# 0xPolygonZero/plonky2

Hardware: NVIDIA H100
Metric: goldilocks_field_elements_per_s_ntt_lde_merkle (higher is better)
Workload: dtype u64

## Files before the change

### plonky2_b200/csrc/gl_lazy.cuh

```cuda
#pragma once
#include "gl_field.cuh"

namespace gl {

struct L3 {
    uint32_t w0, w1;
    int32_t e;
};

GL_HD L3 l3_from(uint64_t x) { return L3{(uint32_t)x, (uint32_t)(x >> 32), 0}; }

#if defined(__CUDA_ARCH__)
__device__ __forceinline__ L3 l3_add(L3 a, L3 b) {
    L3 r;
    asm("add.cc.u32 %0, %3, %6;\n\taddc.cc.u32 %1, %4, %7;\n\taddc.u32 %2, %5, %8;"
        : "=r"(r.w0), "=r"(r.w1), "=r"(r.e)
        : "r"(a.w0), "r"(a.w1), "r"(a.e), "r"(b.w0), "r"(b.w1), "r"(b.e));
    return r;
}
__device__ __forceinline__ L3 l3_sub(L3 a, L3 b) {
    L3 r;
    asm("sub.cc.u32 %0, %3, %6;\n\tsubc.cc.u32 %1, %4, %7;\n\tsubc.u32 %2, %5, %8;"
        : "=r"(r.w0), "=r"(r.w1), "=r"(r.e)
        : "r"(a.w0), "r"(a.w1), "r"(a.e), "r"(b.w0), "r"(b.w1), "r"(b.e));
// ... 66 lines not shown
    return r;
}
inline L3 l3_add(L3 a, L3 b) { return l3_of(l3_val(a) + l3_val(b)); }
inline L3 l3_sub(L3 a, L3 b) { return l3_of(l3_val(a) - l3_val(b)); }
inline uint64_t l3_norm(L3 a) {
    __int128 v = l3_val(a) % (__int128)P;
    if (v < 0) v += P;
    return (uint64_t)v;
}
template <int S>
inline L3 l3_shift(L3 a) { return l3_from(mul_pow2(l3_norm(a), (uint32_t)S)); }
#endif

template <int S>
GL_HD L3 l3_shift_c(L3 a) { return l3_shift<S>(a); }
template <int M, int L, int B>
struct DftLazyBfly {
    static GL_HD void run(L3* r) {
        constexpr int half = 1 << (M - 1 - L);
        constexpr int j = B % half, blk = (B / half) * 2 * half;
        constexpr int sh = (96 / half) * j;
        const L3 u = r[blk + j], v = r[blk + j + half];
        r[blk + j] = l3_add(u, v);
        r[blk + j + half] = l3_shift_c<sh>(l3_sub(u, v));
        if constexpr (B + 1 < (1 << (M - 1))) DftLazyBfly<M, L, B + 1>::run(r);
        else if constexpr (L + 1 < M) DftLazyBfly<M, L + 1, 0>::run(r);
    }
};
template <int M>
GL_HD void dft_lazy(L3* r) {
    if constexpr (M > 0) DftLazyBfly<M, 0, 0>::run(r);
}

}
```

### plonky2_b200/csrc/gl_ntt.cuh

```cuda
#pragma once
#include "gl_lazy.cuh"

namespace gl {

constexpr int NTT_MAX_LOG_PASS = 10;
constexpr int NTT_COL_MIN_LOG = 5;

GL_HD constexpr int ntt_r2(int log) { return log / 2; }
GL_HD constexpr int ntt_r1(int log) { return log - log / 2; }

template <int LOG>
struct PassCfg {
    static constexpr int R1 = ntt_r1(LOG), R2 = ntt_r2(LOG);
    static constexpr int E = 1 << R1, TPT = 1 << R2, NSUB = E / TPT;
    static constexpr int ROW_THREADS = (TPT * 8 < 32) ? 32 : TPT * 8;
    static constexpr int LPC = ROW_THREADS / TPT;
    static constexpr int ROW_MIN_BLOCKS = (E >= 32 ? 512 : 768) / ROW_THREADS;
    static constexpr int ROW_PITCH = TPT + 1;
    static constexpr int ROW_S_WORDS = E * ROW_PITCH;
    static constexpr int GATHER_PITCH = (1 << LOG) + 2;
    static constexpr int T = (256 / TPT) < 8 ? 8 : (256 / TPT);
    static constexpr int COL_THREADS = T * TPT;
    static constexpr int COL_MIN_BLOCKS = (E >= 32 ? 512 : 768) / COL_THREADS;
    static constexpr int COL_QPITCH = TPT * T + 8;
    static constexpr int COL_S_WORDS = E * COL_QPITCH;
};
GL_HD constexpr size_t ntt_row_smem_bytes(int log, bool natural) {
    const int r1 = ntt_r1(log), r2 = ntt_r2(log), E = 1 << r1, TPT = 1 << r2;
    const int threads = (TPT * 8 < 32) ? 32 : TPT * 8, lpc = threads / TPT;
    const size_t s = (size_t)lpc * E * (TPT + 1), g = natural ? (size_t)lpc * ((1 << log) + 2) : 0;
    return (s > g ? s : g) * 8;
}
GL_HD constexpr size_t ntt_col_smem_bytes(int log) {
    const int r1 = ntt_r1(log), r2 = ntt_r2(log), E = 1 << r1, TPT = 1 << r2;
    const int T = (256 / TPT) < 8 ? 8 : (256 / TPT);
    return (size_t)E * (TPT * T + 8) * 8;
}

GL_HD uint64_t table_step_entry(int log, uint32_t idx, uint64_t scale, uint64_t base) {
    const int r1 = ntt_r1(log), r2 = ntt_r2(log);
    const uint32_t t = idx & ((1u << r2) - 1), q = idx >> r2;
    const uint64_t k = bitrev32(q, (uint32_t)r1);
    uint64_t v = pow(root_of_unity((uint32_t)log), k * t);
    if (base != 1) v = mul(v, pow(base, t));
    if (scale != 1) v = mul(v, scale);
    return v;
}
GL_HD uint64_t table_post_entry(int a, int b, size_t idx, uint64_t base) {
    const size_t p = idx >> b, j2 = idx & (((size_t)1 << b) - 1);
    const uint64_t k1 = bitrev32((uint32_t)p, (uint32_t)a);
    uint64_t v = pow(root_of_unity((uint32_t)(a + b)), k1 * j2);
    if (base != 1) v = mul(v, pow(base, j2));
    return v;
}

template <int LOG>
GL_HD void pass_step1(uint64_t* x, const uint64_t* tw, const uint64_t* uq, bool tw_full, int t) {
    using Cf = PassCfg<LOG>;
    L3 r[Cf::E];
#pragma unroll
    for (int q = 0; q < Cf::E; q++) {
        uint64_t v = x[q];
// ... 105 lines not shown
    return cp.twa + (p << cp.log_c) + (size_t)tile * Cf::T + tt;
}
template <int LOG>
GL_HD void col_phase2_store(const ColPass& cp, int blk, int tid, const uint64_t* z, const uint64_t* tws, size_t stride_j,
                            size_t stride_m) {
    using Cf = PassCfg<LOG>;
    const int tt = tid % Cf::T, t = tid / Cf::T;
    size_t in_off, out_off;
    int tile;
    col_unit<LOG>(cp, blk, in_off, out_off, tile);
    const size_t C = (size_t)1 << cp.log_c;
    uint64_t* dst = cp.out + out_off + (size_t)tile * Cf::T + tt;
#pragma unroll
    for (int m = 0; m < Cf::NSUB; m++) {
#pragma unroll
        for (int j = 0; j < Cf::TPT; j++) {
            const int i = m * Cf::TPT + j;
            const size_t p = (size_t)(t + Cf::TPT * m) * Cf::TPT + j;
            dst[p * C] = mul(z[i], tws[m * stride_m + j * stride_j]);
        }
    }
}
template <int LOG>
GL_HD void col_phase2(const ColPass& cp, const uint64_t* S, int blk, int tid) {
    using Cf = PassCfg<LOG>;
    if (Cf::R2 == 0) return;
    uint64_t z[Cf::E];
    col_phase2_load<LOG>(S, tid, z);
    col_phase2_dft<LOG>(z);
    const size_t C = (size_t)1 << cp.log_c;
    col_phase2_store<LOG>(cp, blk, tid, z, col_twiddle_src<LOG>(cp, blk, tid, 0), C, (size_t)Cf::TPT * Cf::TPT * C);
}

enum RowMode { RM_BITREV = 0, RM_NATURAL = 1 };
struct RowPass {
    const uint64_t* in;
    uint64_t* out;
    size_t in_stride, out_stride;
    const uint64_t* tw;
    int log_r;
    int ncols;
    int tw_full;
    int has_uq;
    int reverse;
    size_t row0;
    int n_peer;
    uint64_t* out_peer[7];
    uint64_t uq[32];
};
template <int LOG, int MODE>
GL_HD bool row_line(const RowPass& rp, int blk, int l, size_t& col, size_t& prow, size_t& kbase) {
    using Cf = PassCfg<LOG>;
    const size_t L = (size_t)blk * Cf::LPC + l;
    const size_t R = (size_t)1 << rp.log_r;
    col = L >> rp.log_r;
    const size_t low = L & (R - 1);
    if (MODE == RM_BITREV) {
        prow = low;
        kbase = 0;
    } else {
        kbase = low;
        prow = rp.log_r ? (size_t)bitrev32((uint32_t)low, (uint32_t)rp.log_r) : 0;
    }
    return col < (size_t)rp.ncols;
}
template <int LOG>
GL_HD int row_blocks(const RowPass& rp) {
    using Cf = PassCfg<LOG>;
    const size_t lines = (size_t)rp.ncols << rp.log_r;
    return (int)((lines + Cf::LPC - 1) / Cf::LPC);
}
template <int LOG, int MODE>
GL_HD void row_load(const RowPass& rp, int blk, int tid, uint64_t* x) {
    using Cf = PassCfg<LOG>;
    const int l = tid / Cf::TPT, t = tid % Cf::TPT;
    size_t col, prow, kbase;
    const bool live = row_line<LOG, MODE>(rp, blk, l, col, prow, kbase);
    const uint64_t* src = rp.in + col * rp.in_stride + (prow << LOG) + t;
#pragma unroll
    for (int q = 0; q < Cf::E; q++) x[q] = live ? src[Cf::TPT * q] : 0;
}
template <int LOG, int MODE>
GL_HD void row_phase1(const RowPass& rp, uint64_t* S, int blk, int tid, uint64_t* x) {
    using Cf = PassCfg<LOG>;
    const int l = tid / Cf::TPT, t = tid % Cf::TPT;
    pass_step1<LOG>(x, rp.tw, rp.has_uq ? rp.uq : nullptr, rp.tw_full != 0, t);
    if (Cf::R2 == 0) return;
    uint64_t* Sl = S + (size_t)l * Cf::ROW_S_WORDS;
#pragma unroll
    for (int q = 0; q < Cf::E; q++) Sl[q * Cf::ROW_PITCH + t] = x[q];
}
template <int LOG>
GL_HD uint32_t row_natural_index(int q, int j) {
    using Cf = PassCfg<LOG>;
    return bitrev32((uint32_t)q, Cf::R1) + (uint32_t)Cf::E * (Cf::R2 ? bitrev32((uint32_t)j, Cf::R2) : 0u);
}
template <int LOG>
GL_HD void row_phase2_load(const uint64_t* S, int tid, int m, uint64_t* z) {
    using Cf = PassCfg<LOG>;
    const int l = tid / Cf::TPT, t = tid % Cf::TPT;
    const uint64_t* Sl = S + (size_t)l * Cf::ROW_S_WORDS;
    const int q = t + Cf::TPT * m;
#pragma unroll
// ... 139 lines not shown
```

### plonky2_b200/csrc/gl_ntt_host.cuh

```cuda
#pragma once

template <int LOG, bool ASYNC_TW>
__global__ void __launch_bounds__(PassCfg<LOG>::COL_THREADS, PassCfg<LOG>::COL_MIN_BLOCKS) k_ntt_col(ColPass cp) {
    using Cf = PassCfg<LOG>;
    extern __shared__ __align__(16) u64 smem[];
    u64* tw_s = smem;
    u64* S = smem + (1 << LOG);
    u64* mbar = S + Cf::COL_S_WORDS;
    tma_table_issue(tw_s, cp.tw, (uint32_t)((1 << LOG) * 8), mbar);
    u64 x[Cf::E];
    col_load<LOG>(cp, blockIdx.x, threadIdx.x, x);
    __syncthreads();
    ColPass c2 = cp;
    c2.tw = tw_s;
    tma_table_wait(mbar);
    col_phase1<LOG>(c2, S, blockIdx.x, threadIdx.x, x);
    if (Cf::R2 == 0) return;
    __syncthreads();
    if (!ASYNC_TW) {
        col_phase2<LOG>(c2, S, blockIdx.x, threadIdx.x);
        return;
    }
    col_phase2_load<LOG>(S, threadIdx.x, x);
    __syncthreads();
// ... 48 lines not shown
            if (!(q == 0 && skip0)) y = mul(y, twp[(size_t)q * tws]);
            x[q] = y;
        }
        if (s == 0) {
#pragma unroll
            for (int q = 0; q < Cf::E; q++) S[q * Cf::COL_QPITCH + t * Cf::T + tt] = x[q];
            __syncthreads();
#pragma unroll
            for (int j = 0; j < Cf::TPT; j++) x[j] = S[t * Cf::COL_QPITCH + j * Cf::T + tt];
            skip0 = false;
            const u64* tw2 = cp.twa + (((size_t)t * Cf::TPT) << cp.log_c) + (size_t)tile * Cf::T + tt;
            if (ASYNC_TW) {
                __syncthreads();
#pragma unroll
                for (int j = 0; j < Cf::TPT; j++)
                    asm volatile("cp.async.ca.shared.global [%0], [%1], 8;" ::"r"(smem_u32(S + col_twiddle_slot<LOG>(threadIdx.x, j))),
                                 "l"(tw2 + (size_t)j * C)
                                 : "memory");
                asm volatile("cp.async.commit_group;" ::: "memory");
                twp = S + col_twiddle_slot<LOG>(threadIdx.x, 0);
                tws = Cf::COL_THREADS;
            } else {
                twp = tw2;
                tws = C;
            }
        }
    }
    u64* dst = cp.out + out_off + (size_t)tile * Cf::T + tt;
#pragma unroll
    for (int j = 0; j < Cf::TPT; j++) dst[((size_t)t * Cf::TPT + j) * C] = x[j];
}

template <int LOG, int MODE>
__global__ void __launch_bounds__(PassCfg<LOG>::ROW_THREADS, PassCfg<LOG>::ROW_MIN_BLOCKS) k_ntt_row(RowPass rp) {
    using Cf = PassCfg<LOG>;
    extern __shared__ __align__(16) u64 smem[];
    u64* tw_s = smem;
    u64* S = smem + (1 << LOG);
    u64* mbar = S + ntt_row_smem_bytes(LOG, MODE == RM_NATURAL) / 8;
    RowPass r2 = rp;
    u64 x[Cf::E];
    if (Cf::R2 > 0 && LOG >= 4) {
        tma_table_issue(tw_s, rp.tw, (uint32_t)((1 << LOG) * 8), mbar);
        row_load<LOG, MODE>(rp, blockIdx.x, threadIdx.x, x);
        __syncthreads();
        r2.tw = tw_s;
        tma_table_wait(mbar);
    } else {
        row_load<LOG, MODE>(rp, blockIdx.x, threadIdx.x, x);
    }
    row_phase1<LOG, MODE>(r2, S, blockIdx.x, threadIdx.x, x);
    if (Cf::R2 == 0) {
        if (MODE == RM_BITREV) {
            row_store_bitrev<LOG>(r2, blockIdx.x, threadIdx.x, 0, x);
        } else {
            row_gather_write<LOG>(S, threadIdx.x, 0, x);
            __syncthreads();
            row_store_natural<LOG>(r2, S, blockIdx.x, threadIdx.x, blockDim.x);
        }
        return;
    }
    __syncwarp();
    if (MODE == RM_BITREV) {
#pragma unroll
        for (int m = 0; m < Cf::NSUB; m++) {
            u64 z[Cf::TPT];
            row_phase2_load<LOG>(S, threadIdx.x, m, z);
            pass_step2<LOG>(z);
            row_store_bitrev<LOG>(r2, blockIdx.x, threadIdx.x, m, z);
        }
    } else {
        u64 z[Cf::NSUB][Cf::TPT];
#pragma unroll
        for (int m = 0; m < Cf::NSUB; m++) {
            row_phase2_load<LOG>(S, threadIdx.x, m, z[m]);
            pass_step2<LOG>(z[m]);
        }
        __syncthreads();
#pragma unroll
        for (int m = 0; m < Cf::NSUB; m++) row_gather_write<LOG>(S, threadIdx.x, m, z[m]);
        __syncthreads();
        row_store_natural<LOG>(r2, S, blockIdx.x, threadIdx.x, blockDim.x);
    }
}

template <int LOG, int MODE>
__global__ void __launch_bounds__(PassCfg<LOG>::ROW_THREADS, PassCfg<LOG>::ROW_MIN_BLOCKS) k_ntt_row_shared(RowPass rp) {
    using Cf = PassCfg<LOG>;
    static_assert(Cf::E == Cf::TPT && Cf::R2 > 0 && LOG >= 4, "shared-body row pass needs an even LOG >= 4");
    extern __shared__ __align__(16) u64 smem[];
    u64* tw_s = smem;
    u64* S = smem + (1 << LOG);
    u64* mbar = S + ntt_row_smem_bytes(LOG, MODE == RM_NATURAL) / 8;
    u64 x[Cf::E];
    tma_table_issue(tw_s, rp.tw, (uint32_t)((1 << LOG) * 8), mbar);
    row_load<LOG, MODE>(rp, blockIdx.x, threadIdx.x, x);
    __syncthreads();
    tma_table_wait(mbar);
    const int l = threadIdx.x / Cf::TPT, t = threadIdx.x % Cf::TPT;
    u64* Sl = S + (size_t)l * Cf::ROW_S_WORDS;
    if (rp.has_uq) {
#pragma unroll
        for (int q = 1; q < Cf::E; q++) x[q] = mul(x[q], rp.uq[q]);
    }
    const bool skip0 = rp.tw_full == 0;
    bool do_mul = true;
#pragma unroll 1
    for (int s = 0; s < 2; s++) {
        L3 r[Cf::E];
#pragma unroll
        for (int q = 0; q < Cf::E; q++) r[q] = l3_from(x[q]);
        dft_lazy<Cf::R1>(r);
#pragma unroll
        for (int q = 0; q < Cf::E; q++) {
            u64 y = l3_norm(r[q]);
            if (do_mul && !(q == 0 && skip0)) y = mul(y, tw_s[q * Cf::TPT + t]);
            x[q] = y;
        }
        if (s == 0) {
#pragma unroll
            for (int q = 0; q < Cf::E; q++) Sl[q * Cf::ROW_PITCH + t] = x[q];
            __syncwarp();
#pragma unroll
            for (int j = 0; j < Cf::TPT; j++) x[j] = Sl[t * Cf::ROW_PITCH + j];
            do_mul = false;
        }
    }
    if (MODE == RM_BITREV) {
        row_store_bitrev<LOG>(rp, blockIdx.x, threadIdx.x, 0, x);
    } else {
        __syncthreads();
        row_gather_write<LOG>(S, threadIdx.x, 0, x);
        __syncthreads();
        row_store_natural<LOG>(rp, S, blockIdx.x, threadIdx.x, blockDim.x);
    }
}

__global__ void k_fill_step(int log, u64 scale, u64 base, u64* out) {
    uint32_t j = blockIdx.x * blockDim.x + threadIdx.x;
    if (j < (1u << log)) out[j] = table_step_entry(log, j, scale, base);
}
__global__ void k_fill_post(int a, int b, u64 base, u64* out) {
    size_t i = (size_t)blockIdx.x * blockDim.x + threadIdx.x;
    if (i < ((size_t)1 << (a + b))) out[i] = table_post_entry(a, b, i, base);
}
__global__ void k_fill_pows(const u64* bases, int ntab, size_t count, u64* out) {
    size_t i = (size_t)blockIdx.x * blockDim.x + threadIdx.x;
    if (i >= count * ntab) return;
    size_t t = i / count, e = i % count;
    out[i] = gl::pow(bases[t], e);
}
__global__ void k_mul_pows(u64* data, size_t stride, size_t n, const u64* hi, const u64* lo, int lowbits) {
    size_t k = (size_t)blockIdx.x * blockDim.x + threadIdx.x;
    if (k >= n) return;
    u64* col = data + (size_t)blockIdx.y * stride;
    u64 f = mul(hi[k >> lowbits], lo[k & (((size_t)1 << lowbits) - 1)]);
    col[k] = canon(mul(col[k], f));
}

template <int LOG>
static int launch_col(gl_ctx* ctx, const ColPass& cp, size_t ncols) {
    const int nblocks = col_blocks<LOG>(cp, ncols);
    const size_t smem = ((size_t)(1 << LOG) + PassCfg<LOG>::COL_S_WORDS) * 8 + 16;
    auto go = [&](auto kern) -> int {
        const void* fn = (const void*)kern;
        if (!ctx->smem_attr_done.count(fn)) {
            CK(ctx, cudaFuncSetAttribute(kern, cudaFuncAttributeMaxDynamicSharedMemorySize, (int)smem));
            CK(ctx, cudaFuncSetAttribute(kern, cudaFuncAttributePreferredSharedMemoryCarveout, cudaSharedmemCarveoutMaxShared));
            ctx->smem_attr_done.insert(fn);
        }
        kern<<<nblocks, PassCfg<LOG>::COL_THREADS, smem, ctx->stream>>>(cp);
        CKL(ctx);
        return GL_OK;
    };
    if constexpr (PassCfg<LOG>::E == PassCfg<LOG>::TPT) {
        if (ctx->ntt_variant == 0) return cp.has_uq ? go(k_ntt_col_shared<LOG, true>) : go(k_ntt_col_shared<LOG, false>);
    }
    return cp.has_uq ? go(k_ntt_col<LOG, true>) : go(k_ntt_col<LOG, false>);
}
template <int LOG, int MODE>
static int launch_row(gl_ctx* ctx, const RowPass& rp) {
    const size_t smem = (size_t)(1 << LOG) * 8 + ntt_row_smem_bytes(LOG, MODE == RM_NATURAL) + 16;
    auto go = [&](auto kern) -> int {
        const void* fn = (const void*)kern;
        if (!ctx->smem_attr_done.count(fn)) {
            CK(ctx, cudaFuncSetAttribute(kern, cudaFuncAttributeMaxDynamicSharedMemorySize, (int)smem));
            CK(ctx, cudaFuncSetAttribute(kern, cudaFuncAttributePreferredSharedMemoryCarveout, cudaSharedmemCarveoutMaxShared));
            ctx->smem_attr_done.insert(fn);
        }
        kern<<<row_blocks<LOG>(rp), PassCfg<LOG>::ROW_THREADS, smem, ctx->stream>>>(rp);
        CKL(ctx);
        return GL_OK;
    };
    if constexpr (PassCfg<LOG>::E == PassCfg<LOG>::TPT && LOG >= 4) {
        if (ctx->ntt_variant == 0) return go(k_ntt_row_shared<LOG, MODE>);
    }
    return go(k_ntt_row<LOG, MODE>);
}
static int dispatch_col(gl_ctx* ctx, int a, const ColPass& cp, size_t ncols) {
    switch (a) {
        case 5: return launch_col<5>(ctx, cp, ncols);
        case 6: return launch_col<6>(ctx, cp, ncols);
        case 7: return launch_col<7>(ctx, cp, ncols);
        case 8: return launch_col<8>(ctx, cp, ncols);
        case 9: return launch_col<9>(ctx, cp, ncols);
        case 10: return launch_col<10>(ctx, cp, ncols);
    }
    return set_err(ctx, GL_ERR_UNSUPPORTED, "column pass log %d", a);
}
static int dispatch_row(gl_ctx* ctx, int b, int mode, const RowPass& rp) {
#define ROW_CASE(L)                                                     \
    case L:                                                             \
        return mode == RM_BITREV ? launch_row<L, RM_BITREV>(ctx, rp) : launch_row<L, RM_NATURAL>(ctx, rp);
    switch (b) {
        ROW_CASE(1) ROW_CASE(2) ROW_CASE(3) ROW_CASE(4) ROW_CASE(5) ROW_CASE(6) ROW_CASE(7) ROW_CASE(8) ROW_CASE(9) ROW_CASE(10)
    }
#undef ROW_CASE
    return set_err(ctx, GL_ERR_UNSUPPORTED, "row pass log %d", b);
}

static void table_cache_trim(gl_ctx* ctx, size_t incoming_bytes) {
    const size_t cap = (size_t)3 << 30;
    if (ctx->table_bytes + incoming_bytes <= cap) return;
    for (auto& kv : ctx->step_tabs) cudaFreeAsync(kv.second, ctx->stream);
    for (auto& kv : ctx->post_tabs) cudaFreeAsync(kv.second, ctx->stream);
    ctx->step_tabs.clear();
    ctx->post_tabs.clear();
    ctx->table_bytes = 0;
// ... 181 lines not shown
```

### include/plonky2_b200.h

```cpp
#ifndef PLONKY2_B200_H
#define PLONKY2_B200_H
#include <stddef.h>
#include <stdint.h>

#ifdef __cplusplus
extern "C" {
#endif

#define GL_OK 0
#define GL_ERR_BAD_SHAPE 1
#define GL_ERR_OOM 2
#define GL_ERR_CUDA 3
#define GL_ERR_UNSUPPORTED 4
#define GL_ERR_BAD_ARG 5
#define GL_ERR_POW_FAILED 6
#define GL_ERR_DIV_ZERO 7

#define GL_MEM_HOST 0
#define GL_MEM_DEVICE 1

#define GL_SALT_SIZE 4

typedef struct gl_ctx gl_ctx;
typedef struct gl_commit gl_commit;
typedef struct gl_merkle gl_merkle;
typedef struct gl_fri gl_fri;

int gl_ctx_create(int device, void* stream, gl_ctx** out);
void gl_ctx_destroy(gl_ctx* ctx);
const char* gl_last_error(const gl_ctx* ctx);
int gl_ctx_synchronize(gl_ctx* ctx);
void* gl_ctx_stream(const gl_ctx* ctx);
uint64_t gl_ctx_launch_count(const gl_ctx* ctx);
int gl_ctx_set_ntt_group(gl_ctx* ctx, uint32_t columns);
#define GL_PHASE_INTT 0
#define GL_PHASE_LDE 1
#define GL_PHASE_LEAF_HASH 2
#define GL_PHASE_MERKLE_LEVELS 3
#define GL_NUM_PHASES 4
int gl_ctx_set_profiling(gl_ctx* ctx, int on);
int gl_ctx_phase_ms(gl_ctx* ctx, int phase, double* ms, uint64_t* count);
int gl_ctx_reset_phases(gl_ctx* ctx);

int gl_ntt(gl_ctx* ctx, uint64_t* data, uint32_t log_n, uint32_t batch, size_t stride, int inverse,
           uint32_t zero_factor_log, uint64_t coset_shift, int mem);

int gl_ntt_bcast(gl_ctx* ctx, const uint64_t* in, size_t in_stride, uint32_t log_n, uint32_t batch, int inverse,
                 uint64_t* const* outs, uint32_t n_outs, size_t out_stride);

int gl_bcast(gl_ctx* ctx, const uint64_t* src, size_t words, uint64_t* const* dests, uint32_t n_dests, uint32_t max_ctas);

int gl_commit_create(gl_ctx* ctx, const uint64_t* cols, size_t col_stride, uint32_t B, uint32_t log_n,
                     uint32_t rate_bits, uint32_t cap_height, const uint64_t* salt, int is_coeffs,
                     int mem, gl_commit** out);
int gl_commit_create_sharded(gl_ctx* ctx, const uint64_t* cols, size_t col_stride, uint32_t B, uint32_t log_n,
                             uint32_t rate_bits, uint32_t cap_height, const uint64_t* salt, int is_coeffs,
                             int mem, uint32_t shard_index, uint32_t num_shards, gl_commit** out);
#define GL_COLS_VALUES 0
#define GL_COLS_COEFFS 1
#define GL_COLS_COEFFS_CANONICAL 2
int gl_commit_begin(gl_ctx* ctx, uint32_t B, uint32_t log_n, uint32_t rate_bits, uint32_t cap_height, int blinding,
                    uint32_t shard_index, uint32_t num_shards, uint64_t* coeff_storage, gl_commit** out);
int gl_commit_add_columns(gl_commit* c, uint32_t first_col, uint32_t count, const uint64_t* cols, size_t col_stride,
                          int kind, int mem);
int gl_commit_finish(gl_commit* c, const uint64_t* salt, int mem);
int gl_commit_finish_keyed(gl_commit* c, const uint8_t key[32]);
int gl_commit_finish_prefixed(gl_commit* c, const uint64_t* prefix);
// ... 165 lines not shown
```

### plonky2_b200/_native.py

```python
import ctypes as C
import os

import numpy as np

HERE = os.path.dirname(os.path.abspath(__file__))
LIB_PATH = os.path.join(HERE, "libplonky2_b200.so")

GL_OK = 0
GL_ERR_BAD_SHAPE, GL_ERR_OOM, GL_ERR_CUDA, GL_ERR_UNSUPPORTED, GL_ERR_BAD_ARG, GL_ERR_POW_FAILED, GL_ERR_DIV_ZERO = 1, 2, 3, 4, 5, 6, 7
MEM_HOST, MEM_DEVICE = 0, 1
COLS_VALUES, COLS_COEFFS, COLS_COEFFS_CANONICAL = 0, 1, 2

u64p = C.POINTER(C.c_uint64)
u32p = C.POINTER(C.c_uint32)
vp = C.c_void_p

EXPORTS = [
    "gl_ctx_create", "gl_ctx_destroy", "gl_last_error", "gl_ctx_synchronize", "gl_ctx_launch_count",
    "gl_ctx_set_ntt_group", "gl_ctx_set_profiling", "gl_ctx_phase_ms", "gl_ctx_reset_phases", "gl_ctx_stream", "gl_ntt",
    "gl_ntt_bcast", "gl_bcast", "gl_commit_create", "gl_commit_create_sharded", "gl_commit_begin", "gl_commit_add_columns",
    "gl_commit_finish", "gl_commit_shard", "gl_commit_destroy", "gl_commit_num_polys",
    "gl_commit_leaf_width", "gl_commit_degree_log", "gl_commit_rate_bits", "gl_commit_cap_height",
    "gl_commit_cap", "gl_commit_coeffs", "gl_commit_leaves", "gl_commit_digests", "gl_commit_get_lde_values",
    "gl_commit_open", "gl_commit_eval_ext", "gl_openings", "gl_openings_shard", "gl_stark_quotient", "gl_stark_quotient_aux", "gl_stark_quotient_shard", "gl_stark_quotient_from_shards", "gl_stark_lookup_helpers", "gl_stark_ctl_helpers", "gl_plonk_quotient", "gl_plonk_quotient_shard", "gl_lookup_polys", "gl_sigma_polys", "gl_commit_dev_lde", "gl_commit_dev_coeffs", "gl_partial_products_and_zs", "gl_poseidon_permute_host",
    "gl_poseidon_permute_many", "gl_poseidon_hash_many", "gl_poseidon_hash_no_pad_many", "gl_poseidon_two_to_one_many", "gl_merkle_build", "gl_merkle_destroy",
    "gl_merkle_cap", "gl_merkle_digests", "gl_merkle_open", "gl_fri_begin", "gl_fri_begin_values", "gl_fri_values_local", "gl_fri_begin_from_coeffs",
    "gl_fri_destroy", "gl_fri_coeffs", "gl_fri_commit_round", "gl_fri_commit_round_sharded", "gl_fri_mix", "gl_fri_fold", "gl_fri_final_poly",
    "gl_fri_open", "gl_fri_num_rounds", "gl_fri_pow", "gl_commit_finish_keyed", "gl_random_field_elements",
    "gl_commit_finish_prefixed", "gl_commit_dev_cap",
]


class FriBatch(C.Structure):
    _fields_ = [("point", C.c_uint64 * 2), ("num_polys", C.c_size_t), ("oracle_index", u32p),
                ("poly_index", u32p)]


class ShapeError(ValueError):
    """Mirrors the reference's shape panics (fft.rs:171-177, merkle_tree.rs:195-200, oracle.rs:128)."""


class NativeError(RuntimeError):
    pass


_lib = None


def lib():
    global _lib
    if _lib is not None:
        return _lib
    if not os.path.exists(LIB_PATH):
        raise NativeError(
            "libplonky2_b200.so is not built (run `python -c 'import __graft_entry__ as g; g.build()'`); "
            "plonky2_b200 has no CPU fallback")
    L = C.CDLL(LIB_PATH)
    L.gl_ctx_create.argtypes = [C.c_int, vp, C.POINTER(vp)]
    L.gl_ctx_destroy.argtypes = [vp]
    L.gl_ctx_destroy.restype = None
    L.gl_last_error.argtypes = [vp]
    L.gl_last_error.restype = C.c_char_p
    L.gl_ctx_synchronize.argtypes = [vp]
    L.gl_ctx_launch_count.argtypes = [vp]
    L.gl_ctx_launch_count.restype = C.c_uint64
    L.gl_ctx_set_ntt_group.argtypes = [vp, C.c_uint32]
    L.gl_ntt.argtypes = [vp, vp, C.c_uint32, C.c_uint32, C.c_size_t, C.c_int, C.c_uint32, C.c_uint64, C.c_int]
    L.gl_ctx_stream.argtypes = [vp]
    L.gl_ctx_stream.restype = vp
    L.gl_ntt_bcast.argtypes = [vp, vp, C.c_size_t, C.c_uint32, C.c_uint32, C.c_int, C.POINTER(vp), C.c_uint32, C.c_size_t]
    L.gl_bcast.argtypes = [vp, vp, C.c_size_t, C.POINTER(vp), C.c_uint32, C.c_uint32]
    L.gl_commit_begin.argtypes = [vp, C.c_uint32, C.c_uint32, C.c_uint32, C.c_uint32, C.c_int, C.c_uint32, C.c_uint32,
                                  vp, C.POINTER(vp)]
    L.gl_commit_add_columns.argtypes = [vp, C.c_uint32, C.c_uint32, vp, C.c_size_t, C.c_int, C.c_int]
    L.gl_commit_finish.argtypes = [vp, vp, C.c_int]
    L.gl_commit_finish_keyed.argtypes = [vp, C.c_char_p]
    L.gl_commit_finish_prefixed.argtypes = [vp, vp]
    L.gl_random_field_elements.argtypes = [vp, C.c_char_p, C.c_uint32, C.c_uint64, C.c_size_t, vp, C.c_int]
    L.gl_commit_create.argtypes = [vp, vp, C.c_size_t, C.c_uint32, C.c_uint32, C.c_uint32, C.c_uint32, vp,
                                   C.c_int, C.c_int, C.POINTER(vp)]
    L.gl_commit_create_sharded.argtypes = [vp, vp, C.c_size_t, C.c_uint32, C.c_uint32, C.c_uint32, C.c_uint32, vp,
                                           C.c_int, C.c_int, C.c_uint32, C.c_uint32, C.POINTER(vp)]
    L.gl_commit_shard.argtypes = [vp, u32p, u32p]
    L.gl_ctx_set_profiling.argtypes = [vp, C.c_int]
    L.gl_ctx_phase_ms.argtypes = [vp, C.c_int, C.POINTER(C.c_double), C.POINTER(C.c_uint64)]
    L.gl_ctx_reset_phases.argtypes = [vp]
    L.gl_commit_destroy.argtypes = [vp]
    L.gl_commit_destroy.restype = None
    for n in ("gl_commit_num_polys", "gl_commit_leaf_width", "gl_commit_degree_log", "gl_commit_rate_bits",
              "gl_commit_cap_height"):
        getattr(L, n).argtypes = [vp]
        getattr(L, n).restype = C.c_uint32
    L.gl_commit_cap.argtypes = [vp, vp, C.c_int]
    L.gl_commit_coeffs.argtypes = [vp, vp, C.c_int]
    L.gl_commit_leaves.argtypes = [vp, C.c_size_t, C.c_size_t, vp, C.c_int]
    L.gl_commit_digests.argtypes = [vp, vp, C.c_int]
    L.gl_commit_get_lde_values.argtypes = [vp, C.c_size_t, C.c_size_t, vp]
    L.gl_commit_open.argtypes = [vp, vp, C.c_size_t, vp, vp]
    L.gl_commit_eval_ext.argtypes = [vp, vp, vp]
# ... 93 lines not shown


class Context(Handle):
    destroyer = "gl_ctx_destroy"
    _torch_stream = None

    def __init__(self, device=0, stream=None):
        h = vp()
        check(lib().gl_ctx_create(int(device), vp(stream) if stream else None, C.byref(h)))
        self.h = h
        self.device = device

    def synchronize(self):
        check(lib().gl_ctx_synchronize(self.h), self.h)

    def after_caller(self):
        import torch

        if self._torch_stream is None:
            self._torch_stream = torch.cuda.ExternalStream(self.stream, device=torch.device("cuda", self.device))
        self._torch_stream.wait_stream(torch.cuda.current_stream(self._torch_stream.device))

    @property
    def stream(self):
        return int(lib().gl_ctx_stream(self.h) or 0)

    @property
    def launch_count(self):
        return int(lib().gl_ctx_launch_count(self.h))

    def set_ntt_group(self, columns):
        check(lib().gl_ctx_set_ntt_group(self.h, int(columns)), self.h)

    PHASES = {"intt": 0, "lde": 1, "leaf_hash": 2, "merkle_levels": 3}

    def set_profiling(self, on):
        check(lib().gl_ctx_set_profiling(self.h, int(bool(on))), self.h)

    def reset_phases(self):
        check(lib().gl_ctx_reset_phases(self.h), self.h)

    def phase_ms(self):
        out = {}
        for name, pid in self.PHASES.items():
            ms, cnt = C.c_double(), C.c_uint64()
            check(lib().gl_ctx_phase_ms(self.h, pid, C.byref(ms), C.byref(cnt)), self.h)
            out[name] = (ms.value, cnt.value)
        return out


_default_ctx = {}


def default_context(device=0):
    if device not in _default_ctx:
        _default_ctx[device] = Context(device)
    return _default_ctx[device]
```

### plonky2_b200/csrc/plonky2_b200.cu

```cuda
#include <cooperative_groups.h>
#include <cub/device/device_radix_sort.cuh>
#include <cuda_runtime.h>

#include <cstdarg>
#include <cstdio>
#include <cstring>
#include <functional>
#include <initializer_list>
#include <map>
#include <memory>
#include <set>
#include <string>
#include <tuple>
#include <vector>

#include <sys/random.h>

#include <cerrno>

#include "../../include/plonky2_b200.h"
#include "gl_chacha.cuh"
#include "gl_field.cuh"
#include "gl_logup.cuh"
#include "gl_ctl.cuh"
#include "gl_ntt.cuh"
#include "gl_poseidon.cuh"
#include "gl_sigma.cuh"
#include "gl_vanishing.cuh"

using namespace gl;
typedef uint64_t u64;

static thread_local std::string g_last_error;

struct gl_ctx {
    int device = 0;
    cudaStream_t stream = nullptr;
    bool own_stream = false;
    u64 launches = 0;
    std::string err;
    std::map<std::tuple<int, u64, u64>, u64*> step_tabs;
    std::map<std::tuple<int, int, u64>, u64*> post_tabs;
    size_t table_bytes = 0;
    std::map<int, u64*> fold_tabs;
    cudaStream_t copy_stream = nullptr;
    std::set<const void*> smem_attr_done;
    u64* scratch = nullptr;
    size_t scratch_words = 0;
    u64* pinned = nullptr;
    size_t pinned_words = 0;
    u64* dstage = nullptr;
    size_t dstage_words = 0;
    uint32_t ntt_group = 0;
    int ntt_variant = 0;
    int sm_count = 0;
    int coop_ok = 0;
    int coop_blocks_per_sm = 0;
    bool prof_on = false;
    struct Pending {
        int phase;
        cudaEvent_t a, b;
    };
    std::vector<Pending> prof_pending;
    double prof_ms[GL_NUM_PHASES] = {0};
    u64 prof_count[GL_NUM_PHASES] = {0};
};

struct PhaseScope {
    gl_ctx* ctx;
    cudaEvent_t a = nullptr, b = nullptr;
    int phase;
    PhaseScope(gl_ctx* c, int ph) : ctx(c), phase(ph) {
        if (!ctx->prof_on) return;
        cudaEventCreate(&a);
        cudaEventCreate(&b);
        cudaEventRecord(a, ctx->stream);
    }
    ~PhaseScope() {
        if (!a) return;
        cudaEventRecord(b, ctx->stream);
        ctx->prof_pending.push_back({phase, a, b});
    }
};

static int set_err(gl_ctx* ctx, int code, const char* fmt, ...) {
    char buf[512];
    va_list ap;
// ... 1415 lines not shown
        delete ctx;
        return rc_init;
    }
    cudaMemPool_t pool;
    if (cudaDeviceGetDefaultMemPool(&pool, device) == cudaSuccess) {
        unsigned long long thr = ~0ULL;
        cudaMemPoolSetAttribute(pool, cudaMemPoolAttrReleaseThreshold, &thr);
    }
    *out = ctx;
    return GL_OK;
}
void gl_ctx_destroy(gl_ctx* ctx) {
    if (!ctx) return;
    cudaSetDevice(ctx->device);
    cudaStreamSynchronize(ctx->stream);
    for (auto& kv : ctx->step_tabs) cudaFreeAsync(kv.second, ctx->stream);
    for (auto& kv : ctx->post_tabs) cudaFreeAsync(kv.second, ctx->stream);
    for (auto& kv : ctx->fold_tabs) cudaFreeAsync(kv.second, ctx->stream);
    if (ctx->copy_stream) cudaStreamDestroy(ctx->copy_stream);
    if (ctx->scratch) cudaFreeAsync(ctx->scratch, ctx->stream);
    if (ctx->dstage) cudaFreeAsync(ctx->dstage, ctx->stream);
    if (ctx->pinned) cudaFreeHost(ctx->pinned);
    cudaStreamSynchronize(ctx->stream);
    if (ctx->own_stream) cudaStreamDestroy(ctx->stream);
    delete ctx;
}
const char* gl_last_error(const gl_ctx* ctx) { return ctx ? ctx->err.c_str() : g_last_error.c_str(); }
int gl_ctx_synchronize(gl_ctx* ctx) {
    CK(ctx, cudaStreamSynchronize(ctx->stream));
    return GL_OK;
}
uint64_t gl_ctx_launch_count(const gl_ctx* ctx) { return ctx->launches; }
int gl_ctx_set_ntt_group(gl_ctx* ctx, uint32_t columns) {
    ctx->ntt_variant = (columns >> 31) & 1;
    ctx->ntt_group = columns & 0x7FFFFFFFu;
    return GL_OK;
}
int gl_ctx_set_profiling(gl_ctx* ctx, int on) {
    ctx->prof_on = on != 0;
    return GL_OK;
}
int gl_ctx_phase_ms(gl_ctx* ctx, int phase, double* ms, uint64_t* count) {
    if (phase < 0 || phase >= GL_NUM_PHASES) return set_err(ctx, GL_ERR_BAD_ARG, "bad phase");
    if (!ctx->prof_pending.empty()) {
        CK(ctx, cudaStreamSynchronize(ctx->stream));
        for (auto& p : ctx->prof_pending) {
            float t = 0;
            cudaEventElapsedTime(&t, p.a, p.b);
            ctx->prof_ms[p.phase] += t;
            ctx->prof_count[p.phase]++;
            cudaEventDestroy(p.a);
            cudaEventDestroy(p.b);
        }
        ctx->prof_pending.clear();
    }
    if (ms) *ms = ctx->prof_ms[phase];
    if (count) *count = ctx->prof_count[phase];
    return GL_OK;
}
int gl_ctx_reset_phases(gl_ctx* ctx) {
    TRY(gl_ctx_phase_ms(ctx, 0, nullptr, nullptr));
    for (int i = 0; i < GL_NUM_PHASES; i++) {
        ctx->prof_ms[i] = 0;
        ctx->prof_count[i] = 0;
    }
    return GL_OK;
}

// ... 1528 lines not shown
```

Before: 8.050 billion.

## Run row-pass radix DFT butterflies in FP64 limb pairs instead of integer L3

Adds a P2 representation that holds each Goldilocks element as two double-precision 32-bit limbs. The radix-32 shift butterflies of the shared-body row pass use FMA-based splitting in this form, then normalise back to a u64. It is enabled only for bitrev row passes with R1==R2>=5, where the row thread count per line is halved (4 instead of 8 per TPT) and the launch bounds minimum blocks change. This moves butterfly work from the integer carry-chain pipes onto the FP64 units. The cost is extra registers, since each element now takes two doubles, and correctness rests on proven limb bounds for at most 5 levels.

```diff
diff --git a/plonky2_b200/csrc/gl_lazy.cuh b/plonky2_b200/csrc/gl_lazy.cuh
--- a/plonky2_b200/csrc/gl_lazy.cuh
+++ b/plonky2_b200/csrc/gl_lazy.cuh
@@ -122,4 +122,101 @@
     if constexpr (M > 0) DftLazyBfly<M, 0, 0>::run(r);
 }
 
-}
+#if !defined(GL_NTT_TRACK)
+#define GL_NTT_TRACK(x)
+#endif
+struct P2 {
+    double l, h;
+};
+GL_HD double p2_bits(uint32_t lo, uint32_t hi) {
+#if defined(__CUDA_ARCH__)
+    return __hiloint2double((int)hi, (int)lo);
+#else
+    const uint64_t b = ((uint64_t)hi << 32) | lo;
+    double d;
+    __builtin_memcpy(&d, &b, 8);
+    return d;
+#endif
+}
+GL_HD uint64_t p2_word_bits(double x) {
+#if defined(__CUDA_ARCH__)
+    return (uint64_t)__double_as_longlong(x);
+#else
+    uint64_t b;
+    __builtin_memcpy(&b, &x, 8);
+    return b;
+#endif
+}
+GL_HD double p2_fma(double a, double b, double c) {
+#if defined(__CUDA_ARCH__)
+    return fma(a, b, c);
+#else
+    return __builtin_fma(a, b, c);
+#endif
+}
+GL_HD P2 p2_from(uint64_t x) {
+    return P2{p2_bits((uint32_t)x, 0x43300000u) - 4503599627370496.0, p2_bits((uint32_t)(x >> 32), 0x43300000u) - 4503599627370496.0};
+}
+GL_HD P2 p2_add(P2 a, P2 b) {
+    const P2 o{a.l + b.l, a.h + b.h};
+    GL_NTT_TRACK(o.l);
+    GL_NTT_TRACK(o.h);
+    return o;
+}
+GL_HD P2 p2_sub(P2 a, P2 b) {
+    const P2 o{a.l - b.l, a.h - b.h};
+    GL_NTT_TRACK(o.l);
+    GL_NTT_TRACK(o.h);
+    return o;
+}
+template <int S>
+GL_HD P2 p2_shift(P2 a) {
+    static_assert(S >= 0 && S < 96, "shift out of range");
+    constexpr int q = S / 32, r = S % 32;
+    if constexpr (S == 0) return a;
+    const double C84 = 29014219670751100192948224.0;
+    const double I32 = 2.3283064365386962890625e-10;
+    const double TR = (double)(1u << r);
+    const double lh = p2_fma(a.l, TR, C84) - C84, hh = p2_fma(a.h, TR, C84) - C84;
+    const double ll = p2_fma(a.l, TR, -lh), hl = p2_fma(a.h, TR, -hh);
+    P2 o;
+    if constexpr (q == 0) {
+        o.l = p2_fma(hh, -I32, ll);
+        o.h = p2_fma(hh, I32, p2_fma(lh, I32, hl));
+    } else if constexpr (q == 1) {
+        o.l = p2_fma(hh, -I32, p2_fma(lh, -I32, -hl));
+        o.h = p2_fma(lh, I32, ll + hl);
+    } else {
+        o.l = p2_fma(lh, -I32, -(ll + hl));
+        o.h = p2_fma(hh, -I32, ll);
+    }
+    GL_NTT_TRACK(o.l);
+    GL_NTT_TRACK(o.h);
+    return o;
+}
+GL_HD uint64_t p2_norm(P2 a) {
+    const uint64_t bl = p2_word_bits(a.l + (6755399441055744.0 + 524288.0));
+    const uint64_t bh = p2_word_bits(a.h + (6755399441055744.0 - 1048576.0));
+    const uint64_t s = ((bl >> 32) & 0xFFFFFu) + (bh & 0xFFFFFFFFu);
+    return reduce96((s << 32) | (bl & 0xFFFFFFFFu), (uint32_t)((bh >> 32) & 0xFFFFFu) + (uint32_t)(s >> 32));
+}
+template <int M, int L, int B>
+struct DftPairBfly {
+    static GL_HD void run(P2* r) {
+        constexpr int half = 1 << (M - 1 - L);
+        constexpr int j = B % half, blk = (B / half) * 2 * half;
+        constexpr int sh = (96 / half) * j;
+        const P2 u = r[blk + j], v = r[blk + j + half];
+        r[blk + j] = p2_add(u, v);
+        r[blk + j + half] = p2_shift<sh>(p2_sub(u, v));
+        if constexpr (B + 1 < (1 << (M - 1))) DftPairBfly<M, L, B + 1>::run(r);
+        else if constexpr (L + 1 < M) DftPairBfly<M, L + 1, 0>::run(r);
+    }
+};
+template <int M>
+GL_HD void dft_pair(P2* r) {
+    static_assert(M <= 5, "limb bounds are proved for at most 5 levels");
+    if constexpr (M > 0) DftPairBfly<M, 0, 0>::run(r);
+}
+
+}
diff --git a/plonky2_b200/csrc/gl_ntt.cuh b/plonky2_b200/csrc/gl_ntt.cuh
--- a/plonky2_b200/csrc/gl_ntt.cuh
+++ b/plonky2_b200/csrc/gl_ntt.cuh
@@ -8,6 +8,19 @@
 
 GL_HD constexpr int ntt_r2(int log) { return log / 2; }
 GL_HD constexpr int ntt_r1(int log) { return log - log / 2; }
+
+enum RowMode { RM_BITREV = 0, RM_NATURAL = 1 };
+#if defined(__CUDACC__) && !defined(GL_NTT_ROW_L3)
+constexpr bool NTT_ROW_FP64 = true;
+#else
+constexpr bool NTT_ROW_FP64 = false;
+#endif
+GL_HD constexpr bool ntt_row_pairs(int log, int mode) {
+    return NTT_ROW_FP64 && mode == RM_BITREV && ntt_r1(log) >= 5 && ntt_r1(log) == ntt_r2(log);
+}
+GL_HD constexpr int ntt_row_threads(int log, int mode) {
+    return ((1 << ntt_r2(log)) * (ntt_row_pairs(log, mode) ? 4 : 8) < 32) ? 32 : (1 << ntt_r2(log)) * (ntt_row_pairs(log, mode) ? 4 : 8);
+}
 
 template <int LOG>
 struct PassCfg {
@@ -25,9 +38,15 @@
     static constexpr int COL_QPITCH = TPT * T + 8;
     static constexpr int COL_S_WORDS = E * COL_QPITCH;
 };
+template <int LOG, int MODE>
+struct RowGeom {
+    static constexpr int THREADS = ntt_row_threads(LOG, MODE);
+    static constexpr int LPC = THREADS / PassCfg<LOG>::TPT;
+    static constexpr int MIN_BLOCKS = ntt_row_pairs(LOG, MODE) ? 384 / THREADS : PassCfg<LOG>::ROW_MIN_BLOCKS;
+};
 GL_HD constexpr size_t ntt_row_smem_bytes(int log, bool natural) {
     const int r1 = ntt_r1(log), r2 = ntt_r2(log), E = 1 << r1, TPT = 1 << r2;
-    const int threads = (TPT * 8 < 32) ? 32 : TPT * 8, lpc = threads / TPT;
+    const int threads = ntt_row_threads(log, natural ? RM_NATURAL : RM_BITREV), lpc = threads / TPT;
     const size_t s = (size_t)lpc * E * (TPT + 1), g = natural ? (size_t)lpc * ((1 << log) + 2) : 0;
     return (s > g ? s : g) * 8;
 }
@@ -199,7 +218,6 @@
     col_phase2_store<LOG>(cp, blk, tid, z, col_twiddle_src<LOG>(cp, blk, tid, 0), C, (size_t)Cf::TPT * Cf::TPT * C);
 }
 
-enum RowMode { RM_BITREV = 0, RM_NATURAL = 1 };
 struct RowPass {
     const uint64_t* in;
     uint64_t* out;
@@ -217,8 +235,7 @@
 };
 template <int LOG, int MODE>
 GL_HD bool row_line(const RowPass& rp, int blk, int l, size_t& col, size_t& prow, size_t& kbase) {
-    using Cf = PassCfg<LOG>;
-    const size_t L = (size_t)blk * Cf::LPC + l;
+    const size_t L = (size_t)blk * RowGeom<LOG, MODE>::LPC + l;
     const size_t R = (size_t)1 << rp.log_r;
     col = L >> rp.log_r;
     const size_t low = L & (R - 1);
@@ -231,11 +248,11 @@
     }
     return col < (size_t)rp.ncols;
 }
-template <int LOG>
+template <int LOG, int MODE = RM_NATURAL>
 GL_HD int row_blocks(const RowPass& rp) {
-    using Cf = PassCfg<LOG>;
+    constexpr int LPC = RowGeom<LOG, MODE>::LPC;
     const size_t lines = (size_t)rp.ncols << rp.log_r;
-    return (int)((lines + Cf::LPC - 1) / Cf::LPC);
+    return (int)((lines + LPC - 1) / LPC);
 }
 template <int LOG, int MODE>
 GL_HD void row_load(const RowPass& rp, int blk, int tid, uint64_t* x) {
diff --git a/plonky2_b200/csrc/gl_ntt_host.cuh b/plonky2_b200/csrc/gl_ntt_host.cuh
--- a/plonky2_b200/csrc/gl_ntt_host.cuh
+++ b/plonky2_b200/csrc/gl_ntt_host.cuh
@@ -104,7 +104,7 @@
 }
 
 template <int LOG, int MODE>
-__global__ void __launch_bounds__(PassCfg<LOG>::ROW_THREADS, PassCfg<LOG>::ROW_MIN_BLOCKS) k_ntt_row(RowPass rp) {
+__global__ void __launch_bounds__(RowGeom<LOG, MODE>::THREADS, RowGeom<LOG, MODE>::MIN_BLOCKS) k_ntt_row(RowPass rp) {
     using Cf = PassCfg<LOG>;
     extern __shared__ __align__(16) u64 smem[];
     u64* tw_s = smem;
@@ -157,7 +157,7 @@
 }
 
 template <int LOG, int MODE>
-__global__ void __launch_bounds__(PassCfg<LOG>::ROW_THREADS, PassCfg<LOG>::ROW_MIN_BLOCKS) k_ntt_row_shared(RowPass rp) {
+__global__ void __launch_bounds__(RowGeom<LOG, MODE>::THREADS, RowGeom<LOG, MODE>::MIN_BLOCKS) k_ntt_row_shared(RowPass rp) {
     using Cf = PassCfg<LOG>;
     static_assert(Cf::E == Cf::TPT && Cf::R2 > 0 && LOG >= 4, "shared-body row pass needs an even LOG >= 4");
     extern __shared__ __align__(16) u64 smem[];
@@ -179,15 +179,28 @@
     bool do_mul = true;
 #pragma unroll 1
     for (int s = 0; s < 2; s++) {
-        L3 r[Cf::E];
-#pragma unroll
-        for (int q = 0; q < Cf::E; q++) r[q] = l3_from(x[q]);
-        dft_lazy<Cf::R1>(r);
-#pragma unroll
-        for (int q = 0; q < Cf::E; q++) {
-            u64 y = l3_norm(r[q]);
-            if (do_mul && !(q == 0 && skip0)) y = mul(y, tw_s[q * Cf::TPT + t]);
-            x[q] = y;
+        if constexpr (ntt_row_pairs(LOG, MODE)) {
+            P2 r[Cf::E];
+#pragma unroll
+            for (int q = 0; q < Cf::E; q++) r[q] = p2_from(x[q]);
+            dft_pair<Cf::R1>(r);
+#pragma unroll
+            for (int q = 0; q < Cf::E; q++) {
+                u64 y = p2_norm(r[q]);
+                if (do_mul && !(q == 0 && skip0)) y = mul(y, tw_s[q * Cf::TPT + t]);
+                x[q] = y;
+            }
+        } else {
+            L3 r[Cf::E];
+#pragma unroll
+            for (int q = 0; q < Cf::E; q++) r[q] = l3_from(x[q]);
+            dft_lazy<Cf::R1>(r);
+#pragma unroll
+            for (int q = 0; q < Cf::E; q++) {
+                u64 y = l3_norm(r[q]);
+                if (do_mul && !(q == 0 && skip0)) y = mul(y, tw_s[q * Cf::TPT + t]);
+                x[q] = y;
+            }
         }
         if (s == 0) {
 #pragma unroll
@@ -260,7 +273,7 @@
             CK(ctx, cudaFuncSetAttribute(kern, cudaFuncAttributePreferredSharedMemoryCarveout, cudaSharedmemCarveoutMaxShared));
             ctx->smem_attr_done.insert(fn);
         }
-        kern<<<row_blocks<LOG>(rp), PassCfg<LOG>::ROW_THREADS, smem, ctx->stream>>>(rp);
+        kern<<<row_blocks<LOG, MODE>(rp), RowGeom<LOG, MODE>::THREADS, smem, ctx->stream>>>(rp);
         CKL(ctx);
         return GL_OK;
     };
```

New measurement: 8.091 billion (median of 6 runs). About the same (+0.5%).

## Add persistent pipelined column NTT kernel with cp.async prefetch of next tile

Applied to the files above, without the earlier changes.

Introduces a persistent-grid column-pass NTT kernel that loops over blocks and uses cp.async to prefetch the next tile's input, and optionally the second-stage twiddles, into shared memory while the current tile is computed. The grid is sized to the resident CTA count from an occupancy query, with an optional user cap through a new set_ntt_grid API. It is selected by default for even-LOG column passes when the input is 16-byte aligned. The aim is to hide global load latency, at the cost of extra shared memory and possibly lower occupancy.

```diff
diff --git a/include/plonky2_b200.h b/include/plonky2_b200.h
--- a/include/plonky2_b200.h
+++ b/include/plonky2_b200.h
@@ -33,6 +33,7 @@
 void* gl_ctx_stream(const gl_ctx* ctx);
 uint64_t gl_ctx_launch_count(const gl_ctx* ctx);
 int gl_ctx_set_ntt_group(gl_ctx* ctx, uint32_t columns);
+int gl_ctx_set_ntt_grid(gl_ctx* ctx, uint32_t ctas);
 #define GL_PHASE_INTT 0
 #define GL_PHASE_LDE 1
 #define GL_PHASE_LEAF_HASH 2
diff --git a/plonky2_b200/_native.py b/plonky2_b200/_native.py
--- a/plonky2_b200/_native.py
+++ b/plonky2_b200/_native.py
@@ -17,7 +17,7 @@
 
 EXPORTS = [
     "gl_ctx_create", "gl_ctx_destroy", "gl_last_error", "gl_ctx_synchronize", "gl_ctx_launch_count",
-    "gl_ctx_set_ntt_group", "gl_ctx_set_profiling", "gl_ctx_phase_ms", "gl_ctx_reset_phases", "gl_ctx_stream", "gl_ntt",
+    "gl_ctx_set_ntt_group", "gl_ctx_set_ntt_grid", "gl_ctx_set_profiling", "gl_ctx_phase_ms", "gl_ctx_reset_phases", "gl_ctx_stream", "gl_ntt",
     "gl_ntt_bcast", "gl_bcast", "gl_commit_create", "gl_commit_create_sharded", "gl_commit_begin", "gl_commit_add_columns",
     "gl_commit_finish", "gl_commit_shard", "gl_commit_destroy", "gl_commit_num_polys",
     "gl_commit_leaf_width", "gl_commit_degree_log", "gl_commit_rate_bits", "gl_commit_cap_height",
@@ -65,6 +65,7 @@
     L.gl_ctx_launch_count.argtypes = [vp]
     L.gl_ctx_launch_count.restype = C.c_uint64
     L.gl_ctx_set_ntt_group.argtypes = [vp, C.c_uint32]
+    L.gl_ctx_set_ntt_grid.argtypes = [vp, C.c_uint32]
     L.gl_ntt.argtypes = [vp, vp, C.c_uint32, C.c_uint32, C.c_size_t, C.c_int, C.c_uint32, C.c_uint64, C.c_int]
     L.gl_ctx_stream.argtypes = [vp]
     L.gl_ctx_stream.restype = vp
@@ -224,6 +225,9 @@
     def set_ntt_group(self, columns):
         check(lib().gl_ctx_set_ntt_group(self.h, int(columns)), self.h)
 
+    def set_ntt_grid(self, ctas):
+        check(lib().gl_ctx_set_ntt_grid(self.h, int(ctas)), self.h)
+
     PHASES = {"intt": 0, "lde": 1, "leaf_hash": 2, "merkle_levels": 3}
 
     def set_profiling(self, on):
diff --git a/plonky2_b200/csrc/gl_ntt_host.cuh b/plonky2_b200/csrc/gl_ntt_host.cuh
--- a/plonky2_b200/csrc/gl_ntt_host.cuh
+++ b/plonky2_b200/csrc/gl_ntt_host.cuh
@@ -208,6 +208,132 @@
     }
 }
 
+__device__ __forceinline__ void cp_async16(u64* dst, const u64* src) {
+    asm volatile("cp.async.cg.shared.global [%0], [%1], 16;" ::"r"(smem_u32(dst)), "l"(src) : "memory");
+}
+__device__ __forceinline__ void cp_async_commit() { asm volatile("cp.async.commit_group;" ::: "memory"); }
+template <int N>
+__device__ __forceinline__ void cp_async_wait() { asm volatile("cp.async.wait_group %0;" ::"n"(N) : "memory"); }
+
+template <int LOG, int R0, int R1>
+__device__ __forceinline__ void col_prefetch(const ColPass& cp, int blk, u64* P) {
+    using Cf = PassCfg<LOG>;
+    constexpr int CPR = Cf::T / 2, ROWS = Cf::COL_THREADS / CPR;
+    static_assert((R1 - R0) % ROWS == 0, "whole rounds");
+    const int row = R0 + (int)threadIdx.x / CPR, w = (int)threadIdx.x % CPR * 2;
+    const size_t C = (size_t)1 << cp.log_c;
+    size_t in_off, out_off;
+    int tile;
+    col_unit<LOG>(cp, blk, in_off, out_off, tile);
+    const u64* src = cp.in + in_off + (size_t)tile * Cf::T + (size_t)row * C + w;
+    u64* dst = P + (row - R0) * Cf::T + w;
+#pragma unroll 1
+    for (int i = 0; i < (R1 - R0) / ROWS; i++, src += ROWS * C, dst += ROWS * Cf::T) cp_async16(dst, src);
+}
+template <int LOG>
+__host__ __device__ constexpr int col_pipe_x_rows(bool async_tw) { return async_tw ? (1 << LOG) / 2 : 0; }
+template <int LOG>
+__host__ __device__ constexpr size_t col_pipe_smem_bytes(bool async_tw) {
+    return ((size_t)(1 << LOG) + PassCfg<LOG>::COL_S_WORDS + (size_t)col_pipe_x_rows<LOG>(async_tw) * PassCfg<LOG>::T) * 8 +
+           16;
+}
+
+template <int LOG, bool ASYNC_TW>
+__global__ void __launch_bounds__(PassCfg<LOG>::COL_THREADS, PassCfg<LOG>::COL_MIN_BLOCKS)
+    k_ntt_col_pipe(ColPass cp, int nblocks) {
+    using Cf = PassCfg<LOG>;
+    static_assert(Cf::E == Cf::TPT, "pipelined column pass needs an even LOG");
+    constexpr int R = 1 << LOG, XR = col_pipe_x_rows<LOG>(ASYNC_TW);
+    extern __shared__ __align__(16) u64 smem[];
+    u64* tw_s = smem;
+    u64* S = smem + R;
+    u64* X = S + Cf::COL_S_WORDS;
+    u64* mbar = X + XR * Cf::T;
+    tma_table_issue(tw_s, cp.tw, (uint32_t)(R * 8), mbar);
+    if (ASYNC_TW) col_prefetch<LOG, 0, XR>(cp, blockIdx.x, X);
+    col_prefetch<LOG, XR, R>(cp, blockIdx.x, S);
+    cp_async_commit();
+    __syncthreads();
+    tma_table_wait(mbar);
+    const int tt = threadIdx.x % Cf::T, t = threadIdx.x / Cf::T;
+    const size_t C = (size_t)1 << cp.log_c;
+    for (int blk = blockIdx.x; blk < nblocks; blk += gridDim.x) {
+        const int next = blk + gridDim.x;
+        cp_async_wait<0>();
+        __syncthreads();
+        u64 x[Cf::E];
+#pragma unroll
+        for (int q = 0; q < Cf::E; q++) {
+            const int row = t + Cf::TPT * q;
+            x[q] = row < XR ? X[row * Cf::T + tt] : S[(row - XR) * Cf::T + tt];
+        }
+        if (cp.has_uq) {
+#pragma unroll
+            for (int q = 1; q < Cf::E; q++) x[q] = mul(x[q], cp.uq[q]);
+        }
+        const u64* twp = tw_s + t;
+        size_t tws = Cf::TPT;
+        bool skip0 = cp.tw_full == 0;
+#pragma unroll 1
+        for (int s = 0; s < 2; s++) {
+            L3 r[Cf::E];
+#pragma unroll
+            for (int q = 0; q < Cf::E; q++) r[q] = l3_from(x[q]);
+            dft_lazy<Cf::R1>(r);
+            if (ASYNC_TW && s == 1) cp_async_wait<1>();
+#pragma unroll
+            for (int q = 0; q < Cf::E; q++) {
+                u64 y = l3_norm(r[q]);
+                if (!(q == 0 && skip0)) y = mul(y, twp[(size_t)q * tws]);
+                x[q] = y;
+            }
+            if (s == 0) {
+                __syncthreads();
+#pragma unroll
+                for (int q = 0; q < Cf::E; q++) S[q * Cf::COL_QPITCH + t * Cf::T + tt] = x[q];
+                __syncthreads();
+#pragma unroll
+                for (int j = 0; j < Cf::TPT; j++) x[j] = S[t * Cf::COL_QPITCH + j * Cf::T + tt];
+                skip0 = false;
+                size_t in_off, out_off;
+                int tile;
+                col_unit<LOG>(cp, blk, in_off, out_off, tile);
+                const u64* tw2 = cp.twa + (((size_t)t * Cf::TPT) << cp.log_c) + (size_t)tile * Cf::T + tt;
+                __syncthreads();
+                if (ASYNC_TW) {
+#pragma unroll
+                    for (int j = 0; j < Cf::TPT; j++) {
+                        asm volatile("cp.async.ca.shared.global [%0], [%1], 8;" ::"r"(smem_u32(S + col_twiddle_slot<LOG>(threadIdx.x, j))),
+                                     "l"(tw2 + (size_t)j * C)
+                                     : "memory");
+                    }
+                    cp_async_commit();
+                    if (next < nblocks) col_prefetch<LOG, 0, XR>(cp, next, X);
+                    cp_async_commit();
+                    twp = S + col_twiddle_slot<LOG>(threadIdx.x, 0);
+                    tws = Cf::COL_THREADS;
+                } else {
+                    if (next < nblocks) col_prefetch<LOG, 0, R>(cp, next, S);
+                    cp_async_commit();
+                    twp = tw2;
+                    tws = C;
+                }
+            }
+        }
+        if (ASYNC_TW) {
+            __syncthreads();
+            if (next < nblocks) col_prefetch<LOG, XR, R>(cp, next, S);
+            cp_async_commit();
+        }
+        size_t in_off, out_off;
+        int tile;
+        col_unit<LOG>(cp, blk, in_off, out_off, tile);
+        u64* dst = cp.out + out_off + (size_t)tile * Cf::T + tt;
+#pragma unroll
+        for (int j = 0; j < Cf::TPT; j++) dst[((size_t)t * Cf::TPT + j) * C] = x[j];
+    }
+}
+
 __global__ void k_fill_step(int log, u64 scale, u64 base, u64* out) {
     uint32_t j = blockIdx.x * blockDim.x + threadIdx.x;
     if (j < (1u << log)) out[j] = table_step_entry(log, j, scale, base);
@@ -230,23 +356,57 @@
     col[k] = canon(mul(col[k], f));
 }
 
+template <typename K>
+static int ntt_kernel_attrs(gl_ctx* ctx, K kern, size_t smem) {
+    const void* fn = (const void*)kern;
+    if (!ctx->smem_attr_done.count(fn)) {
+        CK(ctx, cudaFuncSetAttribute(kern, cudaFuncAttributeMaxDynamicSharedMemorySize, (int)smem));
+        CK(ctx, cudaFuncSetAttribute(kern, cudaFuncAttributePreferredSharedMemoryCarveout, cudaSharedmemCarveoutMaxShared));
+        ctx->smem_attr_done.insert(fn);
+    }
+    return GL_OK;
+}
+template <typename K>
+static int ntt_pipe_grid(gl_ctx* ctx, K kern, int threads, size_t smem, int nblocks, int* grid) {
+    TRY(ntt_kernel_attrs(ctx, kern, smem));
+    const void* fn = (const void*)kern;
+    auto it = ctx->resident_ctas.find(fn);
+    if (it == ctx->resident_ctas.end()) {
+        int per_sm = 0;
+        CK(ctx, cudaOccupancyMaxActiveBlocksPerMultiprocessor(&per_sm, kern, threads, smem));
+        if (per_sm < 1) return set_err(ctx, GL_ERR_CUDA, "NTT pass kernel cannot be resident (%zu bytes of shared memory)", smem);
+        it = ctx->resident_ctas.emplace(fn, per_sm * ctx->sm_count).first;
+    }
+    int g = it->second < nblocks ? it->second : nblocks;
+    if (ctx->ntt_grid > 0 && (int)ctx->ntt_grid < g) g = (int)ctx->ntt_grid;
+    *grid = g;
+    return GL_OK;
+}
+static bool ntt_pipe_aligned(const u64* in, size_t in_stride) { return (((uintptr_t)in | (in_stride * 8)) & 15) == 0; }
+
 template <int LOG>
 static int launch_col(gl_ctx* ctx, const ColPass& cp, size_t ncols) {
     const int nblocks = col_blocks<LOG>(cp, ncols);
     const size_t smem = ((size_t)(1 << LOG) + PassCfg<LOG>::COL_S_WORDS) * 8 + 16;
     auto go = [&](auto kern) -> int {
-        const void* fn = (const void*)kern;
-        if (!ctx->smem_attr_done.count(fn)) {
-            CK(ctx, cudaFuncSetAttribute(kern, cudaFuncAttributeMaxDynamicSharedMemorySize, (int)smem));
-            CK(ctx, cudaFuncSetAttribute(kern, cudaFuncAttributePreferredSharedMemoryCarveout, cudaSharedmemCarveoutMaxShared));
-            ctx->smem_attr_done.insert(fn);
-        }
+        TRY(ntt_kernel_attrs(ctx, kern, smem));
         kern<<<nblocks, PassCfg<LOG>::COL_THREADS, smem, ctx->stream>>>(cp);
         CKL(ctx);
         return GL_OK;
     };
     if constexpr (PassCfg<LOG>::E == PassCfg<LOG>::TPT) {
-        if (ctx->ntt_variant == 0) return cp.has_uq ? go(k_ntt_col_shared<LOG, true>) : go(k_ntt_col_shared<LOG, false>);
+        if (ctx->ntt_variant == 0 && ntt_pipe_aligned(cp.in, cp.in_stride)) {
+            auto pipe = [&](auto kern, size_t psmem) -> int {
+                int grid;
+                TRY(ntt_pipe_grid(ctx, kern, PassCfg<LOG>::COL_THREADS, psmem, nblocks, &grid));
+                kern<<<grid, PassCfg<LOG>::COL_THREADS, psmem, ctx->stream>>>(cp, nblocks);
+                CKL(ctx);
+                return GL_OK;
+            };
+            return cp.has_uq ? pipe(k_ntt_col_pipe<LOG, true>, col_pipe_smem_bytes<LOG>(true))
+                             : pipe(k_ntt_col_pipe<LOG, false>, col_pipe_smem_bytes<LOG>(false));
+        }
+        if (ctx->ntt_variant != 1) return cp.has_uq ? go(k_ntt_col_shared<LOG, true>) : go(k_ntt_col_shared<LOG, false>);
     }
     return cp.has_uq ? go(k_ntt_col<LOG, true>) : go(k_ntt_col<LOG, false>);
 }
@@ -254,18 +414,13 @@
 static int launch_row(gl_ctx* ctx, const RowPass& rp) {
     const size_t smem = (size_t)(1 << LOG) * 8 + ntt_row_smem_bytes(LOG, MODE == RM_NATURAL) + 16;
     auto go = [&](auto kern) -> int {
-        const void* fn = (const void*)kern;
-        if (!ctx->smem_attr_done.count(fn)) {
-            CK(ctx, cudaFuncSetAttribute(kern, cudaFuncAttributeMaxDynamicSharedMemorySize, (int)smem));
-            CK(ctx, cudaFuncSetAttribute(kern, cudaFuncAttributePreferredSharedMemoryCarveout, cudaSharedmemCarveoutMaxShared));
-            ctx->smem_attr_done.insert(fn);
-        }
+        TRY(ntt_kernel_attrs(ctx, kern, smem));
         kern<<<row_blocks<LOG>(rp), PassCfg<LOG>::ROW_THREADS, smem, ctx->stream>>>(rp);
         CKL(ctx);
         return GL_OK;
     };
     if constexpr (PassCfg<LOG>::E == PassCfg<LOG>::TPT && LOG >= 4) {
-        if (ctx->ntt_variant == 0) return go(k_ntt_row_shared<LOG, MODE>);
+        if (ctx->ntt_variant != 1) return go(k_ntt_row_shared<LOG, MODE>);
     }
     return go(k_ntt_row<LOG, MODE>);
 }
diff --git a/plonky2_b200/csrc/plonky2_b200.cu b/plonky2_b200/csrc/plonky2_b200.cu
--- a/plonky2_b200/csrc/plonky2_b200.cu
+++ b/plonky2_b200/csrc/plonky2_b200.cu
@@ -53,6 +53,8 @@
     size_t dstage_words = 0;
     uint32_t ntt_group = 0;
     int ntt_variant = 0;
+    uint32_t ntt_grid = 0;
+    std::map<const void*, int> resident_ctas;
     int sm_count = 0;
     int coop_ok = 0;
     int coop_blocks_per_sm = 0;
@@ -1534,8 +1536,12 @@
 }
 uint64_t gl_ctx_launch_count(const gl_ctx* ctx) { return ctx->launches; }
 int gl_ctx_set_ntt_group(gl_ctx* ctx, uint32_t columns) {
-    ctx->ntt_variant = (columns >> 31) & 1;
-    ctx->ntt_group = columns & 0x7FFFFFFFu;
+    ctx->ntt_variant = (columns >> 31) ? 1 : ((columns >> 30) & 1) ? 2 : 0;
+    ctx->ntt_group = columns & 0x3FFFFFFFu;
+    return GL_OK;
+}
+int gl_ctx_set_ntt_grid(gl_ctx* ctx, uint32_t ctas) {
+    ctx->ntt_grid = ctas;
     return GL_OK;
 }
 int gl_ctx_set_profiling(gl_ctx* ctx, int on) {
```

After: 8.065 billion before, 8.066 billion after (median of 6 runs). No clear change (+0.0%).
